# erincatto/solver2d

Measured on AMD Instinct MI355X. Metric: contact-constraints x iters/sec, LargePyramid base-200 TGS_Soft, higher is better.
Workload: dtype f32

## Files before the change

include/solver2d_amd.h:

```cpp
#ifndef SOLVER2D_AMD_H
#define SOLVER2D_AMD_H

#include <stdint.h>

#ifdef __cplusplus
extern "C" {
#endif

#define S2AMD_API_VERSION 5

#define S2AMD_OK 0
#define S2AMD_E_INVALID (-1)
#define S2AMD_E_DEVICE (-2)
#define S2AMD_E_NODEVICE (-3)
#define S2AMD_E_STATE (-4)
#define S2AMD_E_CAPACITY (-5)

typedef enum s2amdSolverType
{
	s2amd_solverJacobi = 0,
	s2amd_solverPGS = 1,
	s2amd_solverPGS_NGS = 2,
	s2amd_solverPGS_NGS_Block = 3,
	s2amd_solverPGS_Soft = 4,
// ... 235 lines not shown
int s2amd_world_get_tree(s2amdSolver* solver, int32_t bodyType, s2amdTreeNode* nodes, int32_t nodeCapacity, int32_t* root);
int s2amd_world_set_contacts(s2amdSolver* solver, const int32_t* slots, int32_t count, const s2amdContact* contacts, const s2amdPairState* pairs);
int s2amd_world_download(s2amdSolver* solver, s2amdBody* bodies, int32_t bodyCapacity, s2amdContact* contacts, int32_t contactCapacity,
						 s2amdJoint* joints, int32_t jointCapacity, s2amdShape* shapes, int32_t shapeCapacity, s2amdPairState* pairs, float* origins,
						 int32_t* status);

int s2amd_find_islands(s2amdSolver* solver, const s2amdBody* bodies, int32_t bodyCapacity, const s2amdContact* contacts, int32_t contactCapacity,
					   const s2amdJoint* joints, int32_t jointCapacity, int32_t* islandOfBody, int32_t* islandCount);
int s2amd_color_constraints(s2amdSolver* solver, const s2amdBody* bodies, int32_t bodyCapacity, const s2amdContact* contacts, int32_t contactCapacity,
							int32_t* colorOfContact, int32_t* colorCount, int32_t* rounds);

int s2amd_export_poses(s2amdSolver* solver, void* devicePoses, int32_t capacity);
int s2amd_export_poses_async(s2amdSolver* solver, void* devicePoses, int32_t capacity, int32_t slot);
int s2amd_export_bodies_async(s2amdSolver* solver, void* deviceRecords, int32_t capacity, int32_t slot);
int s2amd_export_wait(s2amdSolver* solver, int32_t slot);

int s2amd_device_alloc(s2amdSolver* solver, uint64_t bytes, void** devicePtr);
int s2amd_device_free(s2amdSolver* solver, void* devicePtr);
int s2amd_device_read(s2amdSolver* solver, void* hostDst, const void* deviceSrc, uint64_t bytes);

int s2amd_get_contact_order(s2amdSolver* solver, int32_t* order, int32_t orderCapacity, int32_t* colorOffsets,
							int32_t colorCapacity, int32_t* constraintCount, int32_t* colorCount);
int s2amd_get_joint_order(s2amdSolver* solver, int32_t* order, int32_t orderCapacity, int32_t* colorOffsets,
						  int32_t colorCapacity, int32_t* jointCount, int32_t* colorCount);
int s2amd_get_writable_bodies(s2amdSolver* solver, uint8_t* writable, int32_t bodyCapacity, int32_t* solverClass);
int s2amd_get_stats(s2amdSolver* solver, s2amdStepStats* stats);
int s2amd_get_strip_owners(s2amdSolver* solver, int32_t* ownerStrip, int32_t* onSeam, int32_t capacity, int32_t* stripCount);
#define S2AMD_RESIDENT_NONE 0
#define S2AMD_RESIDENT_INTERPRETER 1
#define S2AMD_RESIDENT_ISLAND 2
#define S2AMD_RESIDENT_WIDE 3
#define S2AMD_RESIDENT_WIDE_ONLY_LAUNCH 4
int s2amd_get_resident_kernel(s2amdSolver* solver, int32_t* kernel, int32_t* rounds);
int s2amd_variant_family_count(void);
int s2amd_get_variant_family(int32_t family, const char** kernel, const char** keyFields, int32_t* keyLength, int32_t* entryCount);
int s2amd_get_variant_entry(int32_t family, int32_t entry, int32_t* key, int32_t keyCapacity, uint64_t* selections);
int s2amd_measure_dominant(s2amdSolver* solver, const s2amdStepParams* params, int32_t repeats, float* usPerLaunch,
						   int32_t* launchesPerSweep, int32_t* constraintsPerLaunch);
int s2amd_set_option(s2amdSolver* solver, const char* key, int32_t value);

typedef struct s2amdShardedSolver s2amdShardedSolver;
int s2amd_sharded_create(const int32_t* devices, int32_t deviceCount, s2amdShardedSolver** out);
void s2amd_sharded_destroy(s2amdShardedSolver* sharded);
int s2amd_sharded_shard_count(const s2amdShardedSolver* sharded);
s2amdSolver* s2amd_sharded_solver(s2amdShardedSolver* sharded, int32_t shard);
int s2amd_sharded_upload(s2amdShardedSolver* sharded, const s2amdBody* bodies, int32_t bodyCapacity, const s2amdContact* contacts, int32_t contactCapacity,
						 const s2amdJoint* joints, int32_t jointCapacity);
int s2amd_sharded_step(s2amdShardedSolver* sharded, const s2amdStepParams* params);
int s2amd_sharded_step_async(s2amdShardedSolver* sharded, const s2amdStepParams* params);
int s2amd_sharded_wait(s2amdShardedSolver* sharded);
int s2amd_sharded_get_step_ops(s2amdShardedSolver* sharded, int32_t* streamOps, int32_t* hostWaits, int32_t* exchange);
int s2amd_sharded_count_ops(int32_t shards, int32_t exchange, int32_t* streamOps);
int s2amd_sharded_download(s2amdShardedSolver* sharded, s2amdBody* bodies, int32_t bodyCapacity, s2amdContact* contacts, int32_t contactCapacity,
						   s2amdJoint* joints, int32_t jointCapacity);
int s2amd_sharded_read_bodies(s2amdShardedSolver* sharded, int32_t shard, float* records, int32_t bodyCapacity);
int s2amd_sharded_reshard(s2amdShardedSolver* sharded, const s2amdContact* contacts, int32_t contactCapacity, const s2amdJoint* joints, int32_t jointCapacity);
int s2amd_sharded_get_partition(s2amdShardedSolver* sharded, int32_t* shardOfBody, int32_t capacity, int32_t* islandCount, int32_t* reshards);

#ifdef __cplusplus
}
#endif

#endif
```

solver2d_amd/csrc/solver.cpp:

```cpp

#include <atomic>
#include "solver_executor.h"

namespace
{

thread_local std::string g_lastError;
thread_local std::string g_variantMiss;

}

void s2amdVariantMiss(const char* family, const char* fields, const int* key, int n)
{
	if (!g_variantMiss.empty())
	{
		return;
	}
	std::string text = std::string("no ") + family + " variant for {" + fields + "} = {";
	for (int i = 0; i < n; ++i)
	{
		text += (i != 0 ? ", " : "") + std::to_string(key[i]);
	}
	g_variantMiss = text + "}: nothing was launched for that part of the world";
}
// ... 656 lines not shown
	}
	if (entryCount)
	{
		*entryCount = f[family].entries;
	}
	return S2AMD_OK;
}

int s2amd_get_variant_entry(int32_t family, int32_t entry, int32_t* key, int32_t keyCapacity, uint64_t* selections)
{
	VariantFamily f[S2_VARIANT_FAMILIES];
	if (family < 0 || family >= variantFamilies(f) || entry < 0 || entry >= f[family].entries)
	{
		return fail(S2AMD_E_INVALID, "variant family or entry out of range");
	}
	if (key != nullptr && keyCapacity < f[family].keyLength)
	{
		return fail(S2AMD_E_CAPACITY, "key buffer too small");
	}
	int k[S2_VARIANT_KEY_MAX];
	unsigned long long n = 0;
	f[family].read(f[family].list, entry, k, &n);
	for (int i = 0; key != nullptr && i < f[family].keyLength; ++i)
	{
		key[i] = k[i];
	}
	if (selections)
	{
		*selections = n;
	}
	return S2AMD_OK;
}

int s2amd_get_strip_owners(s2amdSolver* s, int32_t* ownerStrip, int32_t* onSeam, int32_t capacity, int32_t* stripCount)
{
	if (!s)
	{
		return fail(S2AMD_E_INVALID, "null solver");
	}
	const IncrementalStrips& m = s->stripInc;
	const int nb = s->bodyCapacity;
	if ((ownerStrip || onSeam) && capacity < nb)
	{
		return fail(S2AMD_E_CAPACITY, "strip owner buffer too small");
	}
	if (stripCount)
	{
		*stripCount = m.valid ? (int)m.stripBodyCount.size() : 0;
	}
	for (int i = 0; i < nb; ++i)
	{
		if (ownerStrip)
		{
			ownerStrip[i] = (m.valid && i < (int)m.ownerStrip.size()) ? m.ownerStrip[(size_t)i] : -1;
		}
		if (onSeam)
		{
			onSeam[i] = -1;
		}
	}
	if (onSeam && m.valid)
	{
		for (size_t sm = 0; sm < m.seamGroupOf.size(); ++sm)
		{
			const int g = m.seamGroupOf[sm];
			if (g < 0)
// ... 353 lines not shown
		s->structureDirty = true;
	}
	else if (strcmp(key, "persist_debug") == 0)
	{
		s->stripsRejected = false;
		s->optPersistDebug = value;
		s->structureDirty = true;
	}
	else if (strcmp(key, "seam_regs") == 0)
	{
		s->optSeamRegs = value != 0;
		s->structureDirty = true;
	}
	else if (strcmp(key, "wide") == 0)
	{
		s->optWide = value != 0;
		s->structureDirty = true;
	}
	else if (strcmp(key, "pair_lanes") == 0)
	{
		s->optPairLanes = value != 0;
		s->structureDirty = true;
	}
	else if (strcmp(key, "strip_slack") == 0)
	{
		s->optStripSlack = value != 0;
		s->structureDirty = true;
	}
	else if (strcmp(key, "strip_retry") == 0)
	{
		s->optStripRetry = value != 0;
		s->structureDirty = true;
	}
	else if (strcmp(key, "persist") == 0)
	{
		s->stripsRejected = false;
		s->optPersist = value != 0;
		s->structureDirty = true;
	}
	else if (strcmp(key, "strip_patience") == 0)
	{
		s->optStripPatience = std::max(0, value);
		s->stripPatienceNow = s->optStripPatience;
		s->stripPatienceSet = true;
	}
	else if (strcmp(key, "near_handoff") == 0)
	{
		s->optNearHandoff = value != 0;
		s->nearHandoffNow = s->optNearHandoff;
	}
	else if (strcmp(key, "strip_adopt") == 0)
	{
		s->optStripAdopt = value != 0;
	}
	else if (strcmp(key, "prebuild_solver") == 0)
	{
		s->optPrebuildSolver = value;
	}
	else if (strcmp(key, "jacobi_persist") == 0)
	{
		s->optJacobiPersist = value != 0;
		s->structureDirty = true;
	}
	else if (strcmp(key, "jacobi_min_constraints") == 0)
	{
		s->optJacobiMinConstraints = std::max(0, value);
// ... 127 lines not shown
```

solver2d_amd/csrc/solver_async.cpp:

```cpp
#include "solver_internal.h"

#include <atomic>
#include <mutex>
#include <thread>

namespace
{
struct DevPool
{
	std::mutex m;
	std::vector<std::pair<void*, size_t>> blocks;
	size_t bytes = 0;
	std::vector<hipStream_t> streams;
	std::vector<std::pair<void*, size_t>> pinned;
};
constexpr int kMaxPoolDevices = 64;
DevPool& devPool()
{
	static DevPool pools[kMaxPoolDevices];
	int device = 0;
	if (hipGetDevice(&device) != hipSuccess || device < 0 || device >= kMaxPoolDevices)
	{
		(void)hipGetLastError();
		device = 0;
// ... 632 lines not shown
	{
		return false;
	}
	if (job->dropped)
	{
		return false;
	}
	const long due = job->requestedAtStep + (long)job->delay;
	if (s->stepCounter < due)
	{
		return false;
	}
	if (job->forced && !job->done.load(std::memory_order_acquire))
	{
		job->delay += 4;
		return false;
	}
	const double t0 = nowMs();
	const double ta0 = t0;
	if (job->worker.joinable())
	{
		job->worker.join();
	}
	s->asyncWaitMs += (float)(nowMs() - t0);
	s2amdSolver* c = job->clone;
	bool ok = job->rc == S2AMD_OK && job->solverType == solverType && !c->structureDirty;
	auto score = [](const s2amdSolver* x) {
		if (x->dStripA.view.groupCount == 0)
		{
			return 0;
		}
		if (x->persistValid && x->persist.maxRoundsA <= S2_STRIP_ROUNDS)
		{
			return (x->persist.maxRoundsA <= 5 && x->persist.maxSeamRounds <= 2) ? 4 : 3;
		}
		return x->persistValid ? 2 : 1;
	};
	if (ok && job->search)
	{
		if (score(c) <= score(s))
		{
			ok = false;
			if (c->stripScaleFound > 0.0f && c->stripScaleFoundFor == s->stripScaleFoundFor)
			{
				s->stripScaleFound = c->stripScaleFound;
			}
		}
		else
		{
			s->stripSearchPause = 256, s->stripSearchNotBefore = 0;
		}
	}
	const bool poolWas = devPoolOn();
	devPoolThread(true);
	ok = ok && replay(c, job->log);
	if (ok && c->watchedCount > 0)
	{
		if (fetchPointCounts(s) != S2AMD_OK)
		{
			ok = false;
		}
		std::vector<ContactChange> flipped;
		for (int i = 0; ok && i < s->contactCapacity; ++i)
		{
			if (c->hContactWatched[(size_t)i] && s->hContactPoints[(size_t)i] > 0 && c->inc.positionOfSlot[(size_t)i] == -1)
			{
				if (c->hContactEdge[(size_t)i] && !c->hContactDead[(size_t)i] && c->stripInc.valid &&
// ... 51 lines not shown
```

solver2d_amd/csrc/solver_internal.h:

```cpp
#pragma once

#include "launch.h"
#include "s2_device.h"

#include "solver2d_amd.h"

#include <algorithm>
#include <chrono>
#include <cmath>
#include <cstdio>
#include <cstdlib>
#include <cstring>
#include <string>
#include <unordered_map>
#include <vector>

int s2amdFail(int code, const std::string& msg);
inline int fail(int code, const std::string& msg) { return s2amdFail(code, msg); }

#define S2_HUB_DEGREE 12
#define S2_COST_STRIP_ROUND_US 1.4f
#define S2_COST_LAUNCH_US 2.0f
#define S2_COST_BATCH_COLOURS 12
#define S2_COST_TAIL_VISIT_US 0.38f
// ... 371 lines not shown
	std::vector<uint8_t> hBodyLive, hBodyStatic;
	DevBuf dOps;
	long placedTotal = 0;
	DevBuf dSeparated;
	DevBuf dPairLog;
	unsigned long long* hostPairLog = nullptr;
	bool pairLogDirty = false;
	DevBuf dShapeBoxes;
	DevBuf dRefitOrder, dStepBack;
	int refitOrderCount = 0;
	int optTreeStream = 1;
	DeviceTrees* trees = nullptr;
	int lastMovedCount = 0;
	DevBuf dSlotBytes;
	std::vector<uint8_t> hSlotBytes;
	bool slotBytesFresh = false;
	std::vector<int32_t> hSeparated;
	int optIncremental = 1;
	int optDefer = 1;
	int optIslandResident = 1;
	int optStripLean = 1;
	int optStageJoints = 1;
	int optSelfContained = 1;
	int optGeneric = 1;
	int optFreeBodyGroups = 1;
	int optPersist = 1;
	int optSeamRegs = 1;
	int optWide = 1;
	int optWideBodyWarm = 0;
	int optSelfContainedStrips = 0;
	int optStripSlack = 1;
	int optPairLanes = 0;
	int optStripRetry = 1;
	int optPersistDebug = 0;
	int optPersistSpinLimit = 1 << 21;
	bool persistFailed = false;
	int persistFallbacks = 0;
	int optPersistRetry = 256;
	int persistRetryAfter = 256, persistFailedAge = 0;
	int cuCount = 0;
	HubCosts hubCosts;
	unsigned int* hostError = nullptr;
	unsigned long long* hostTimes = nullptr;
	int optMessage = 0;
	int optBodyWarm = 1;
	bool indexInWire = false;
	int graphAge = 0;
	int optStripPatience = 1;
	int optNearHandoff = 1, nearHandoffNow = 1, nearHandoffTimeouts = 0;
	int optStripAdopt = 1;
	int optJacobiPersist = 1;
	int optJacobiMinConstraints = 1024;
	int optOverflow = 1;
	long slicedSteps = 0;
	bool slicedThisStep = false;
	int stripPatienceNow = 1;
	int groupPatienceNow = 0;
	bool dirtyByGroups = false;
	int tailSlackShift = 0;
	bool dirtyByWatched = false;
	int optGroupPatience = 1;
	int optTailTinyColour = 32;
	int optGroupTinyColour = 3;
	int optGenericPlace = 1;
	int optFlipColours = 1;
	bool stripPatienceSet = false;
// ... 166 lines not shown
```

solver2d_amd/csrc/solver_structure.cpp:

```cpp
#include "solver_internal.h"

#include <atomic>

namespace
{

constexpr int ColorBitsWords = 4;

struct Carver
{
	char* p;
	char* end;
	template <class T> T* take(size_t count)
	{
		char* r = p;
		p += (count * sizeof(T) + 255) & ~size_t(255);
		return (T*)r;
	}
};

int growFamily(s2amdSolver* s, DevBuf& buf, int& cap, int need, size_t slotBytes, int arrays)
{
	if (need <= cap && buf.p != nullptr)
	{
// ... 382 lines not shown
	return S2AMD_OK;
}

struct LocalSlots
{
	std::vector<int> slot, stamp;
	int epoch = 0;
	explicit LocalSlots(int nb) : slot((size_t)nb, -1), stamp((size_t)nb, -1) {}
	void begin() { epoch += 1; }
	void seed(int body, std::vector<int>& ids, bool owned)
	{
		stamp[body] = epoch;
		slot[body] = (int)ids.size();
		ids.push_back((int)((uint32_t)body | (owned ? S2G_OWNED : 0u)));
	}
	int get(int body, std::vector<int>& ids, const std::vector<uint8_t>& conflict)
	{
		if (stamp[body] != epoch)
		{
			stamp[body] = epoch;
			slot[body] = (int)ids.size();
			ids.push_back((int)((uint32_t)body | (conflict[body] ? S2G_OWNED : 0u)));
		}
		return slot[body];
	}
};

struct StripPartition
{
	bool active = false;
	std::vector<std::vector<int>> bodies;
	std::vector<std::vector<int>> cA, jA;
	std::vector<std::vector<int>> cB, jB;
};

void partitionStrips(const EdgeList& ce, const EdgeList& je, const std::vector<int>& cGlobal, const std::vector<int>& jGlobal,
					 const std::vector<uint8_t>& conflict, const std::vector<uint8_t>& loose, int nb, int targetBodies, int maxBodies,
					 StripPartition& out)
{
	auto linked = [&](int a, int b) { return a >= 0 && b >= 0 && conflict[a] && conflict[b] && loose[a] && loose[b]; };
	std::vector<int> deg((size_t)nb + 1, 0);
	auto countEdges = [&](const EdgeList& e, const std::vector<int>& ks) {
		for (int k : ks)
		{
			if (linked(e.a[k], e.b[k]))
			{
				deg[(size_t)e.a[k] + 1] += 1;
				deg[(size_t)e.b[k] + 1] += 1;
			}
		}
	};
	countEdges(ce, cGlobal);
	countEdges(je, jGlobal);
	for (int i = 0; i < nb; ++i)
	{
		deg[(size_t)i + 1] += deg[i];
	}
	std::vector<int> adj((size_t)deg[nb]), cursor(deg.begin(), deg.end() - 1);
	auto fillEdges = [&](const EdgeList& e, const std::vector<int>& ks) {
		for (int k : ks)
		{
			if (linked(e.a[k], e.b[k]))
			{
				adj[(size_t)cursor[e.a[k]]++] = e.b[k];
				adj[(size_t)cursor[e.b[k]]++] = e.a[k];
			}
		}
	};
	fillEdges(ce, cGlobal);
	fillEdges(je, jGlobal);

	std::vector<int> level((size_t)nb, -1), queue, levelOffsets{0}, levelBodies;
	std::vector<int> seen((size_t)nb, 0);
	int epoch = 0;
	auto bfs = [&](int root, bool record) {
		epoch += 1;
		queue.clear();
		queue.push_back(root);
		seen[root] = epoch;
		size_t head = 0, levelEnd = 1;
		while (head < queue.size())
		{
			if (head == levelEnd)
			{
				if (record)
				{
					levelOffsets.push_back((int)levelBodies.size());
				}
				levelEnd = queue.size();
			}
			int u = queue[head++];
			if (record)
			{
				level[u] = (int)levelOffsets.size() - 1;
				levelBodies.push_back(u);
			}
			for (int e = deg[u]; e < deg[(size_t)u + 1]; ++e)
			{
				int v = adj[(size_t)e];
				if (seen[v] != epoch)
				{
					seen[v] = epoch;
					queue.push_back(v);
				}
			}
		}
		if (record)
		{
			levelOffsets.push_back((int)levelBodies.size());
		}
		return queue.back();
	};
	for (int i = 0; i < nb; ++i)
	{
		if (!loose[i] || level[i] >= 0)
		{
			continue;
		}
		int far = deg[(size_t)i + 1] > deg[i] ? bfs(i, false) : i;
		bfs(far, true);
	}
	const int levels = (int)levelOffsets.size() - 1;
	if (levels < 4)
	{
		return;
	}

	std::vector<int> stripOf((size_t)nb, -1);
	int curLevels = 0;
	out.bodies.emplace_back();
	for (int l = 0; l < levels; ++l)
	{
		if (curLevels >= 2 && (int)out.bodies.back().size() >= targetBodies)
		{
			out.bodies.emplace_back();
			curLevels = 0;
		}
		for (int e = levelOffsets[l]; e < levelOffsets[(size_t)l + 1]; ++e)
		{
			out.bodies.back().push_back(levelBodies[(size_t)e]);
		}
		curLevels += 1;
	}
	if (curLevels < 2 && out.bodies.size() >= 2)
	{
		std::vector<int> lastStrip = std::move(out.bodies.back());
		out.bodies.pop_back();
		out.bodies.back().insert(out.bodies.back().end(), lastStrip.begin(), lastStrip.end());
	}
	const int K = (int)out.bodies.size();
	if (K < 2)
	{
		out = StripPartition();
		return;
	}
	for (int i = 0; i < K; ++i)
	{
		for (int body : out.bodies[(size_t)i])
		{
			stripOf[body] = i;
		}
	}

	out.cA.assign((size_t)K, {}), out.jA.assign((size_t)K, {});
	out.cB.assign((size_t)K - 1, {}), out.jB.assign((size_t)K - 1, {});
	bool ok = true;
// ... 887 lines not shown
	s2amdSolver* s;
	const int solverType;
	const float stripScale;
	const int cls;
	const bool needAdj;
	const bool grouped;
	const bool ldsGroups;
	const bool wantStrips;
	const bool residentWanted;
	const bool stripSlackWanted;
	const int nb;
	SweepSet& cs;
	SweepSet& js;

	std::vector<uint8_t> conflict;
	EdgeList ce, je;
	int C = 0, J = 0;
	std::vector<int> cPart, jPart;
	int groupCount = 0;
	std::vector<uint32_t> flags;
	std::vector<std::vector<int>> cOf, jOf;
	StripPartition strips;
	bool stripsNeedOneLaunch = false;
	LocalSlots slots;
	std::vector<int> seamGroup;
	struct SpareRound
	{
		int table, group, begin, count, round;
	};
	std::vector<SpareRound> spareRounds;
	int stripBaseC = 0;
	int overflowBase = 0, overflowCount = 0;
	bool rebuild = false;

	double t0, tPhase;
	bool prepTimes;
	double tSlots = 0, tColour = 0, tAppend = 0;

	StructureBuild(s2amdSolver* solver, int type, float scale)
		: s(solver), solverType(type), stripScale(scale), cls(isPositionSolver(type) ? 1 : 0), needAdj(type == s2amd_solverJacobi),
		  grouped(solver->optGroups != 0 && !needAdj),
		  ldsGroups(grouped && (solver->optGroupPatience == 0 || solver->graphAge >= solver->groupPatienceNow)),
		  wantStrips(grouped && solver->optStrips != 0 && !solver->stripsRejected && solver->graphAge >= solver->stripPatienceNow &&
					 (solver->optStripsAnySolver != 0 || isSoftFamily(type) || genericWanted(solver))),
		  residentWanted(grouped && isSoftFamily(type) && solver->optIslandResident != 0 && !solver->residentRejected),
		  stripSlackWanted(solver->optStripSlack != 0 && solver->optIncremental != 0 && solver->optPersist != 0 &&
						   (type == s2amd_solverTGS_Soft || (solver->optWide != 0 && (type == s2amd_solverSoftStep || type == s2amd_solverPGS_Soft)) ||
							(!isSoftFamily(type) && solver->optGenericPlace != 0 && genericWanted(solver)))),
		  nb(solver->bodyCapacity),
		  cs(solver->contacts), js(solver->joints), slots(solver->bodyCapacity)
	{
		static const bool fromEnv = getenv("S2AMD_DEBUG_PREP") != nullptr;
		prepTimes = fromEnv;
		t0 = tPhase = nowMs();
	}

	static bool genericWanted(const s2amdSolver* solver)
	{
		return solver->optGeneric != 0 && solver->optPersist != 0 && solver->optStripLean != 0 && !solver->persistFailed && solver->hostError != nullptr;
	}

	static int stripBodiesFor(const s2amdSolver* solver, int type)
	{
		const bool ldsSeams = (type == s2amd_solverSoftStep || type == s2amd_solverPGS_Soft) && solver->optWide == 0;
		if (solver->stripBodiesSet || !ldsSeams)
		{
// ... 265 lines not shown
			for (int k = 0; k < J; ++k)
			{
				jPart[k] = assign(jRoot[k]);
			}
		}

		phase("islands and groups");
	}

	void splitParts()
	{
		cOf.assign((size_t)groupCount + 1, {}), jOf.assign((size_t)groupCount + 1, {});
		for (int k = 0; k < C; ++k)
		{
			cOf[(size_t)cPart[k] + 1].push_back(k);
		}
		for (int k = 0; k < J; ++k)
		{
			jOf[(size_t)jPart[k] + 1].push_back(k);
		}

		cs = SweepSet();
		js = SweepSet();
		cs.colorOffsets.push_back(0);
		js.colorOffsets.push_back(0);
		s->hGroups.clear();
		s->hResident.clear();
		s->hContactTail.clear();
		s->hJointTail.clear();
		s->hStripA.clear();
		s->hStripB.clear();
	}

	void cutStrips()
	{
		strips = StripPartition();
		stripsNeedOneLaunch = false;
		if (wantStrips && (s->optStripsAnySolver != 0 || jOf[0].empty() || genericWanted(s)))
		{
			std::vector<uint8_t> ownedByIsland((size_t)nb, 0);
			auto mark = [&](int body) {
				if (body >= 0 && conflict[body])
				{
					ownedByIsland[body] = 1;
				}
			};
			for (int k = 0; k < C; ++k)
			{
				if (cPart[k] >= 0)
				{
					mark(ce.a[k]), mark(ce.b[k]);
				}
			}
			for (int k = 0; k < J; ++k)
			{
				if (jPart[k] >= 0)
				{
					mark(je.a[k]), mark(je.b[k]);
				}
			}
			std::vector<uint8_t> loose((size_t)nb);
			int looseCount = 0;
			for (int i = 0; i < nb; ++i)
			{
				loose[i] = s->hBodyLive[i] && !s->hBodyStatic[i] && !ownedByIsland[i];
				looseCount += loose[i];
			}
			if (looseCount >= (s->stripMinBodiesSet || s->maxGroupBodiesSet ? s->optStripMinBodies : std::min(s->optStripMinBodies, groupLowerLimit(solverType))))
			{
				partitionStrips(ce, je, cOf[0], jOf[0], conflict, loose, nb, std::max(8, (int)((float)stripBodiesFor(s, solverType) * stripScale)), s->optMaxGroupBodies, strips);
			}
			if (strips.active)
			{
				std::vector<uint8_t> placed((size_t)nb, 0);
				for (const std::vector<int>& list : strips.bodies)
				{
					for (int b : list)
					{
						placed[(size_t)b] = 1;
					}
				}
				bool unfit = false;
				for (const std::vector<std::vector<int>>* lists : {&strips.cA, &strips.cB})
				{
					for (const std::vector<int>& list : *lists)
					{
						for (int k : list)
						{
							unfit = unfit || (ce.a[k] >= 0 && conflict[(size_t)ce.a[k]] && !placed[(size_t)ce.a[k]]) ||
									 (ce.b[k] >= 0 && conflict[(size_t)ce.b[k]] && !placed[(size_t)ce.b[k]]);
						}
					}
				}
				for (const std::vector<std::vector<int>>* lists : {&strips.jA, &strips.jB})
				{
					for (const std::vector<int>& list : *lists)
					{
						for (int k : list)
						{
							unfit = unfit || (je.a[k] >= 0 && conflict[(size_t)je.a[k]] && !placed[(size_t)je.a[k]]) ||
									 (je.b[k] >= 0 && conflict[(size_t)je.b[k]] && !placed[(size_t)je.b[k]]);
						}
					}
// ... 563 lines not shown
		}
		if ((rc = uploadGroupTable(s, s->hGroups, s->dGroups)) != 0 || (rc = uploadGroupTable(s, s->hContactTail, s->dContactTail, s->hContactTail.count() > 0 ? (size_t)(S2_TAIL_BODY_SLACK << s->tailSlackShift) : 0)) != 0 ||
			(rc = uploadGroupTable(s, s->hJointTail, s->dJointTail)) != 0 ||
			(rc = uploadGroupTable(s, s->hStripA, s->dStripA, s->hStripA.count() > 0 ? (size_t)32 * (size_t)(s->hStripA.maxBodies + S2_STRIP_ADOPT_SLACK) : 0)) != 0 ||
			(rc = uploadGroupTable(s, s->hStripB, s->dStripB)) != 0)
		{
			return rc;
		}
		phase("index tables");
		return S2AMD_OK;
	}

	int buildStripTables()
	{
		int rc;
		s->leanAValid = s->leanBValid = false;
		s->persistValid = false;
		s->leanA = StripTableView{};
		s->leanB = StripTableView{};
		if (strips.active && s->optStripLean)
		{
			if ((rc = buildLeanStripTables(s, strips, conflict, seamGroup, stripBaseC, nb)) != 0)
			{
				return rc;
			}
		}

		s->stripsNeedOneLaunch = strips.active && stripsNeedOneLaunch;
		if (stripsNeedOneLaunch)
		{
			s->leanAValid = s->leanBValid = false;
		}
		const bool soft = isSoftFamily(solverType);
		const bool oneLaunch = (soft && s->persistValid) || s->genericValid;
		const bool multiLaunch = !stripsNeedOneLaunch && (s->optStripsAnySolver != 0 || (soft && js.stripCount == 0 && s->leanAValid && s->leanBValid));
		if (strips.active && !oneLaunch && !multiLaunch)
		{
			s->stripsRejected = true;
			s->structureDirty = true;
			rebuild = true;
			return S2AMD_OK;
		}
		phase("strip tables");
		buildStripMirror();
		phase("strip mirror");
		return S2AMD_OK;
	}

	void buildStripMirror()
	{
		IncrementalStrips& m = s->stripInc;
		m = IncrementalStrips{};
		const bool interpreter = !isSoftFamily(solverType);
		if (!strips.active || !stripSlackWanted || !(interpreter ? s->genericValid : s->persistValid) || js.stripCount != 0)
		{
			return;
		}
		m.base = stripBaseC, m.end = stripBaseC + cs.stripCount;
		if (interpreter)
		{
			m.takeOnly = true;
			m.roundLimit[0] = m.roundLimit[1] = 0;
		}
		if (solverType == s2amd_solverSoftStep)
		{
			m.roundLimit[0] = S2_STRIP_ROUNDS, m.roundLimit[1] = 2;
// ... 156 lines not shown
		for (size_t k = 0; k < cs.order.size(); ++k)
		{
			s->slackPositions += cs.order[k] < 0 ? 1 : 0;
		}
		s->slackAtBuild = s->slackPositions;
		s->inc.valid = s->optIncremental != 0 && s->inc.solverClass == cls && !s->msgTablesValid && !s->inc.positionOfSlot.empty();
		s->inc.patches.clear();
		s->orderSolverClass = cls;
		s->orderResident = residentWanted;
		s->orderColourless = needAdj;
		s->orderGrouped = grouped;
		s->orderLdsGroups = ldsGroups;
		if (getenv("S2AMD_DEBUG"))
		{
			int real = 0;
			for (int k = 0; k < cs.globalCount; ++k)
			{
				real += cs.order[(size_t)k] >= 0 ? 1 : 0;
			}
			fprintf(stderr, "[s2amd] structure: global part %d contact positions (%d constraints, %d batches%s), %d joints; %d LDS groups, %d resident, %d strips; loose bodies %d\n",
					cs.globalCount, real, (int)cs.batchOffsets.size() - 1, cs.hasTail ? ", tail" : "", js.globalCount, s->hGroups.count(), s->hResident.count(),
					s->hStripA.count(), s->looseBodies);
		}
		s->residentAllTwoPoints = residentAllTwoPoints(s) ? 1 : 0;
		s->orderStrips = wantStrips;
		s->orderStripBodies = stripBodiesFor(s, solverType);
		s->structureDirty = false;
		s->structureGeneration += 1;
		s->stats.hostPrepMs = (float)(nowMs() - t0);
		return S2AMD_OK;
	}
};

static int buildStructureWith(s2amdSolver* s, int solverType, float stripScale)
{
	StructureBuild build(s, solverType, stripScale);
	if (build.upToDate())
	{
		return S2AMD_OK;
	}
	if (s->worldResident && !s->pointsKnown)
	{
		int rcDead = syncDeadSlots(s);
		if (rcDead)
		{
			return rcDead;
		}
	}
	int rc = build.gatherEdges();
	if (rc)
	{
		return rc;
	}
	build.findIslands();
	build.splitParts();
	build.cutStrips();
	build.phase("strip partition");
	build.colourGlobalPart();
	build.phase("global part");
	build.emitIslandGroups();
	build.emitStrips();
	if ((rc = build.uploadTables()) != 0 || build.rebuild || (rc = build.buildStripTables()) != 0 || build.rebuild)
	{
		return rc ? rc : buildStructureWith(s, solverType, stripScale);
	}
	return build.finish();
}

int buildStructure(s2amdSolver* s, int solverType)
{
	if (asyncBuildsOn(s) && s->optAsyncBuild >= 2 && !s->structureDirty)
	{
		StructureBuild probe(s, solverType, 1.0f);
		if (probe.onlyStripsMissing())
		{
			return asyncRequest(s, solverType, false);
		}
	}
	const uint64_t before = s->structureGeneration;
	{
		const int cls = isPositionSolver(solverType) ? 1 : 0;
		if (s->stripsJudgedForClass != cls)
		{
			s->stripsRejected = s->stripsHopeless = false;
			s->stripsJudgedForClass = cls;
		}
	}
	if (s->stripScaleFoundFor != StructureBuild::stripBodiesFor(s, solverType))
	{
		s->stripScaleFound = 0.0f;
		s->stripScaleFoundFor = StructureBuild::stripBodiesFor(s, solverType);
	}
	const float firstScale = s->stripScaleFound > 0.0f ? s->stripScaleFound : 1.0f;
	int rc = buildStructureWith(s, solverType, firstScale);
	if (rc != S2AMD_OK || s->structureGeneration == before || s->optStripRetry == 0)
	{
		return rc;
	}
	auto outcome = [&]() {
		if (s->persistValid && !s->persist.wideRounds)
		{
			return (s->persist.maxRoundsA <= 5 && s->persist.maxSeamRounds <= 2) ? 3 : 2;
		}
		return (s->persistValid || (s->leanAValid && s->leanBValid)) ? 1 : 0;
	};
	auto satisfied = [&]() {
		if (!StructureBuild::isSoftFamily(solverType))
		{
			return s->dStripA.view.groupCount > 0 && (s->genericValid || outcome() >= 1);
		}
		if (s->joints.stripCount > 0)
		{
			return s->dStripA.view.groupCount > 0 && s->genericValid;
		}
		return outcome() >= (solverType == s2amd_solverTGS_Soft ? 3 : 2);
	};
	const bool triedStrips = s->stripsRejected || s->dStripA.view.groupCount > 0;
	s->stripRetryPending = false;
	auto usable = [&]() { return s->dStripA.view.groupCount > 0 && s->persistValid && s->stripInc.valid; };
	if (s->forcedBuild && (usable() || !triedStrips || s->stripsHopeless))
	{
		return rc;
	}
	if (!s->forcedBuild && (!triedStrips || s->stripsHopeless || satisfied() || (s->stripScaleFound > 0.0f && outcome() >= 2)))
	{
		return rc;
	}
	if (!s->forcedBuild && s->optStripPatience != 0 && s->graphAge < 32)
	{
		s->stripRetryPending = true;
		return rc;
	}
	float bestScale = firstScale;
	int best = outcome();
	const float scales[] = {4.0f, 10.0f, 20.0f, 2.0f, 40.0f, 80.0f, 0.5f};
// ... 29 lines not shown
```

solver2d_amd/hip.py:

```python
import ctypes
import os

import numpy as np

from . import wire

_HERE = os.path.dirname(os.path.abspath(__file__))
LIB_PATH = os.environ.get("S2AMD_LIB") or os.path.join(_HERE, "libs2amd.so")
FAST_LIB_PATH = os.environ.get("S2AMD_FAST_LIB") or os.path.join(_HERE, "libs2amd_fast.so")

EXPORTS = [
    "s2amd_api_version", "s2amd_build_flags", "s2amd_device_count", "s2amd_device_bus_id", "s2amd_last_error", "s2amd_create", "s2amd_destroy",
    "s2amd_solve", "s2amd_upload", "s2amd_step_resident", "s2amd_download", "s2amd_save_bodies",
    "s2amd_restore_bodies", "s2amd_get_contact_order", "s2amd_get_joint_order", "s2amd_get_writable_bodies", "s2amd_get_stats",
    "s2amd_set_option", "s2amd_export_poses", "s2amd_export_poses_async", "s2amd_export_bodies_async", "s2amd_export_wait", "s2amd_measure_dominant", "s2amd_refit_shapes", "s2amd_find_pairs", "s2amd_synchronize", "s2amd_update_contacts", "s2amd_find_islands", "s2amd_color_constraints",
    "s2amd_world_upload", "s2amd_world_step", "s2amd_world_download", "s2amd_world_find_pairs", "s2amd_world_set_contacts",
    "s2amd_device_alloc", "s2amd_device_free", "s2amd_device_read", "s2amd_world_separated", "s2amd_world_download_boxes", "s2amd_world_set_refit_order", "s2amd_world_download_step", "s2amd_world_set_tree", "s2amd_world_get_tree",
    "s2amd_get_strip_owners", "s2amd_get_resident_kernel", "s2amd_variant_family_count", "s2amd_get_variant_family", "s2amd_get_variant_entry",
    "s2amd_sharded_create", "s2amd_sharded_destroy", "s2amd_sharded_shard_count", "s2amd_sharded_solver", "s2amd_sharded_upload", "s2amd_sharded_step",
    "s2amd_sharded_download", "s2amd_sharded_read_bodies", "s2amd_sharded_reshard", "s2amd_sharded_get_partition",
    "s2amd_sharded_step_async", "s2amd_sharded_wait", "s2amd_sharded_get_step_ops", "s2amd_sharded_count_ops",
]

_libs = {}


class S2AmdError(RuntimeError):
    pass


def load(fast=False):
    path = FAST_LIB_PATH if fast else LIB_PATH
    if path in _libs:
        return _libs[path]
    if not os.path.exists(path):
        raise S2AmdError("HIP extension %s is missing: build it with `make -C solver2d_amd/csrc` "
                         "(there is no CPU fallback)" % path)
    L = ctypes.CDLL(path)
    vp, i32 = ctypes.c_void_p, ctypes.c_int32
    L.s2amd_api_version.restype = ctypes.c_int
    L.s2amd_device_count.restype = ctypes.c_int
    L.s2amd_last_error.restype = ctypes.c_char_p
    L.s2amd_build_flags.restype = ctypes.c_char_p
    L.s2amd_create.argtypes = [ctypes.c_int, ctypes.POINTER(vp)]
    L.s2amd_destroy.argtypes = [vp]
    L.s2amd_destroy.restype = None
    L.s2amd_solve.argtypes = [vp, ctypes.POINTER(wire.StepParams), vp, i32, vp, i32, vp, i32]
    L.s2amd_upload.argtypes = [vp, vp, i32, vp, i32, vp, i32]
    L.s2amd_step_resident.argtypes = [vp, ctypes.POINTER(wire.StepParams)]
    L.s2amd_download.argtypes = [vp, vp, i32, vp, i32, vp, i32]
    L.s2amd_save_bodies.argtypes = [vp]
    L.s2amd_restore_bodies.argtypes = [vp]
    L.s2amd_synchronize.argtypes = [vp]
    L.s2amd_get_contact_order.argtypes = [vp, vp, i32, vp, i32, ctypes.POINTER(i32), ctypes.POINTER(i32)]
    L.s2amd_get_joint_order.argtypes = [vp, vp, i32, vp, i32, ctypes.POINTER(i32), ctypes.POINTER(i32)]
    L.s2amd_get_writable_bodies.argtypes = [vp, vp, i32, ctypes.POINTER(i32)]
    L.s2amd_get_strip_owners.argtypes = [vp, vp, vp, i32, ctypes.POINTER(i32)]
    L.s2amd_get_resident_kernel.argtypes = [vp, ctypes.POINTER(i32), ctypes.POINTER(i32)]
    L.s2amd_variant_family_count.restype = ctypes.c_int
    L.s2amd_get_variant_family.argtypes = [i32, ctypes.POINTER(ctypes.c_char_p), ctypes.POINTER(ctypes.c_char_p), ctypes.POINTER(i32), ctypes.POINTER(i32)]
    L.s2amd_get_variant_entry.argtypes = [i32, i32, ctypes.POINTER(i32), i32, ctypes.POINTER(ctypes.c_uint64)]
    L.s2amd_get_stats.argtypes = [vp, ctypes.POINTER(wire.StepStats)]
    L.s2amd_set_option.argtypes = [vp, ctypes.c_char_p, i32]
    L.s2amd_export_poses.argtypes = [vp, vp, i32]
    L.s2amd_export_poses_async.argtypes = [vp, vp, i32, i32]
    L.s2amd_export_bodies_async.argtypes = [vp, vp, i32, i32]
    L.s2amd_export_wait.argtypes = [vp, i32]
    L.s2amd_measure_dominant.argtypes = [vp, ctypes.POINTER(wire.StepParams), i32, ctypes.POINTER(ctypes.c_float),
                                         ctypes.POINTER(i32), ctypes.POINTER(i32)]
    L.s2amd_refit_shapes.argtypes = [vp, vp, i32, vp, i32, vp]
    L.s2amd_find_pairs.argtypes = [vp, vp, i32, vp, i32, vp, vp, i32, vp, i32, vp, i32, ctypes.POINTER(i32)]
    L.s2amd_update_contacts.argtypes = [vp, vp, i32, vp, vp, i32, vp, vp, i32, vp]
    L.s2amd_world_upload.argtypes = [vp, vp, i32, vp, i32, vp, i32, vp, i32, vp, vp]
    L.s2amd_world_step.argtypes = [vp, ctypes.POINTER(wire.StepParams), ctypes.POINTER(wire.WorldStepInfo)]
    L.s2amd_world_find_pairs.argtypes = [vp, vp, i32, ctypes.POINTER(i32)]
    L.s2amd_world_set_contacts.argtypes = [vp, vp, i32, vp, vp]
    L.s2amd_world_separated.argtypes = [vp, vp, i32, ctypes.POINTER(i32)]
    L.s2amd_world_download_boxes.argtypes = [vp, vp, i32]
    L.s2amd_world_set_refit_order.argtypes = [vp, vp, i32]
    L.s2amd_world_set_tree.argtypes = [vp, i32, vp, i32, i32]
    L.s2amd_world_get_tree.argtypes = [vp, i32, vp, i32, ctypes.POINTER(i32)]
    L.s2amd_world_download.argtypes = [vp, vp, i32, vp, i32, vp, i32, vp, i32, vp, vp, vp]
    L.s2amd_device_alloc.argtypes = [vp, ctypes.c_uint64, ctypes.POINTER(vp)]
    L.s2amd_device_free.argtypes = [vp, vp]
    L.s2amd_device_read.argtypes = [vp, vp, vp, ctypes.c_uint64]
    L.s2amd_find_islands.argtypes = [vp, vp, i32, vp, i32, vp, i32, vp, ctypes.POINTER(i32)]
    L.s2amd_color_constraints.argtypes = [vp, vp, i32, vp, i32, vp, ctypes.POINTER(i32), ctypes.POINTER(i32)]
    L.s2amd_sharded_create.argtypes = [vp, i32, ctypes.POINTER(vp)]
    L.s2amd_sharded_destroy.argtypes = [vp]
    L.s2amd_sharded_destroy.restype = None
    L.s2amd_sharded_shard_count.argtypes = [vp]
# ... 283 lines not shown
        existing = np.ascontiguousarray(existing, dtype=np.int32).reshape(-1, 2)
        moved = np.ascontiguousarray(moved, dtype=np.uint8)
        cap = 4096
        while True:
            out = np.zeros((cap, 2), dtype=np.int32)
            n = ctypes.c_int32()
            rc = self._L.s2amd_find_pairs(self._h, wire.as_ptr(bodies), len(bodies), wire.as_ptr(shapes), len(shapes), wire.as_ptr(moved),
                                         wire.as_ptr(existing), len(existing), wire.as_ptr(joints), len(joints), wire.as_ptr(out), cap,
                                         ctypes.byref(n))
            if rc == -5 and n.value > cap:
                cap = n.value
                continue
            self._ck(rc)
            return out[: n.value].copy()

    def _order(self, fn):
        n, nc = ctypes.c_int32(), ctypes.c_int32()
        self._ck(fn(self._h, None, 0, None, 0, ctypes.byref(n), ctypes.byref(nc)))
        order = np.zeros(max(n.value, 1), dtype=np.int32)
        offsets = np.zeros(nc.value + 1, dtype=np.int32)
        self._ck(fn(self._h, order.ctypes.data, len(order), offsets.ctypes.data, len(offsets), ctypes.byref(n), ctypes.byref(nc)))
        return order[: n.value].copy(), offsets

    def contact_order(self):
        return self._order(self._L.s2amd_get_contact_order)

    def strip_owners(self, body_capacity):
        owner = np.full(max(body_capacity, 1), -1, dtype=np.int32)
        seam = np.full(max(body_capacity, 1), -1, dtype=np.int32)
        n = ctypes.c_int32()
        self._ck(self._L.s2amd_get_strip_owners(self._h, owner.ctypes.data, seam.ctypes.data, len(owner), ctypes.byref(n)))
        return owner[:body_capacity], seam[:body_capacity], n.value

    def resident_kernel(self):
        kernel, rounds = ctypes.c_int32(), ctypes.c_int32()
        self._ck(self._L.s2amd_get_resident_kernel(self._h, ctypes.byref(kernel), ctypes.byref(rounds)))
        return kernel.value, rounds.value

    def joint_order(self):
        return self._order(self._L.s2amd_get_joint_order)

    def synchronize(self):
        self._ck(self._L.s2amd_synchronize(self._h))

    def stats(self):
        st = wire.StepStats()
        self._ck(self._L.s2amd_get_stats(self._h, ctypes.byref(st)))
        return {k: getattr(st, k) for k, _ in wire.StepStats._fields_}


class _BorrowedSolver(Solver):

    def __init__(self, L, handle):
        self._L, self._h, self.fast = L, ctypes.c_void_p(handle), False

    def close(self):
        self._h = None


class ShardedSolver:

    def __init__(self, devices, fast=False):
        L = load(fast=fast)
        devs = (ctypes.c_int32 * len(devices))(*[int(d) for d in devices])
        h = ctypes.c_void_p()
        _check(L.s2amd_sharded_create(devs, len(devices), ctypes.byref(h)), L)
# ... 70 lines not shown
```

Baseline: 6.294 billion.

## Add opt-in strip cut candidates that minimise interior coloring rounds

Adds an optional search over alternative strip partitions: second BFS root, thin end strips, and level-first constraint ordering. It keeps whichever candidate needs the fewest interior color rounds without adding seam rounds, aiming to cut the per-iteration round count in the persistent soft kernel. The partition scoring also now favours structures with four or fewer interior rounds. The search costs extra host time at structure build and may force a rebuild. A query API for strip rounds is added.

Result: slower. 6.226 billion (-1.1%).

```diff
diff --git a/include/solver2d_amd.h b/include/solver2d_amd.h
--- a/include/solver2d_amd.h
+++ b/include/solver2d_amd.h
@@ -291,6 +291,7 @@
 #define S2AMD_RESIDENT_WIDE 3
 #define S2AMD_RESIDENT_WIDE_ONLY_LAUNCH 4
 int s2amd_get_resident_kernel(s2amdSolver* solver, int32_t* kernel, int32_t* rounds);
+int s2amd_get_strip_rounds(s2amdSolver* solver, int32_t* interior, int32_t* seam);
 int s2amd_variant_family_count(void);
 int s2amd_get_variant_family(int32_t family, const char** kernel, const char** keyFields, int32_t* keyLength, int32_t* entryCount);
 int s2amd_get_variant_entry(int32_t family, int32_t entry, int32_t* key, int32_t keyCapacity, uint64_t* selections);
diff --git a/solver2d_amd/csrc/solver.cpp b/solver2d_amd/csrc/solver.cpp
--- a/solver2d_amd/csrc/solver.cpp
+++ b/solver2d_amd/csrc/solver.cpp
@@ -712,6 +712,33 @@
 	return S2AMD_OK;
 }
 
+int s2amd_get_strip_rounds(s2amdSolver* s, int32_t* interior, int32_t* seam)
+{
+	if (!s)
+	{
+		return fail(S2AMD_E_INVALID, "null solver");
+	}
+	const HostGroupTable* tables[2] = {&s->hStripA, &s->hStripB};
+	int32_t* out[2] = {interior, seam};
+	for (int t = 0; t < 2; ++t)
+	{
+		int most = 0;
+		for (int g = 0; s->dStripA.view.groupCount > 0 && g < tables[t]->count(); ++g)
+		{
+			most = std::max(most, tables[t]->cBatchOffsets[(size_t)g + 1] - tables[t]->cBatchOffsets[(size_t)g]);
+		}
+		if (s->persistValid && s->dStripA.view.groupCount > 0)
+		{
+			most = std::max(most, t == 0 ? s->persist.maxRoundsA : s->persist.maxSeamRounds);
+		}
+		if (out[t])
+		{
+			*out[t] = most;
+		}
+	}
+	return S2AMD_OK;
+}
+
 int s2amd_get_strip_owners(s2amdSolver* s, int32_t* ownerStrip, int32_t* onSeam, int32_t capacity, int32_t* stripCount)
 {
 	if (!s)
@@ -1131,6 +1158,13 @@
 		s->optStripRetry = value != 0;
 		s->structureDirty = true;
 	}
+	else if (strcmp(key, "strip_cuts") == 0)
+	{
+		s->optStripCuts = value != 0;
+		s->structureDirty = true;
+		s->stripsRejected = false;
+		s->stripScaleFound = 0.0f;
+	}
 	else if (strcmp(key, "persist") == 0)
 	{
 		s->stripsRejected = false;
diff --git a/solver2d_amd/csrc/solver_async.cpp b/solver2d_amd/csrc/solver_async.cpp
--- a/solver2d_amd/csrc/solver_async.cpp
+++ b/solver2d_amd/csrc/solver_async.cpp
@@ -688,7 +688,7 @@
 		}
 		if (x->persistValid && x->persist.maxRoundsA <= S2_STRIP_ROUNDS)
 		{
-			return (x->persist.maxRoundsA <= 5 && x->persist.maxSeamRounds <= 2) ? 4 : 3;
+			return x->persist.maxSeamRounds > 2 || x->persist.maxRoundsA > 5 ? 3 : (x->persist.maxRoundsA > 4 ? 4 : 5);
 		}
 		return x->persistValid ? 2 : 1;
 	};
diff --git a/solver2d_amd/csrc/solver_internal.h b/solver2d_amd/csrc/solver_internal.h
--- a/solver2d_amd/csrc/solver_internal.h
+++ b/solver2d_amd/csrc/solver_internal.h
@@ -427,6 +427,7 @@
 	int optStripSlack = 1;
 	int optPairLanes = 0;
 	int optStripRetry = 1;
+	int optStripCuts = 0;
 	int optPersistDebug = 0;
 	int optPersistSpinLimit = 1 << 21;
 	bool persistFailed = false;
diff --git a/solver2d_amd/csrc/solver_structure.cpp b/solver2d_amd/csrc/solver_structure.cpp
--- a/solver2d_amd/csrc/solver_structure.cpp
+++ b/solver2d_amd/csrc/solver_structure.cpp
@@ -438,11 +438,19 @@
 	std::vector<std::vector<int>> bodies;
 	std::vector<std::vector<int>> cA, jA;
 	std::vector<std::vector<int>> cB, jB;
+	std::vector<int> level;
+};
+
+struct StripCut
+{
+	bool secondRoot = false;
+	bool thinEnds = false;
+	int maxStrips = 0;
 };
 
 void partitionStrips(const EdgeList& ce, const EdgeList& je, const std::vector<int>& cGlobal, const std::vector<int>& jGlobal,
 					 const std::vector<uint8_t>& conflict, const std::vector<uint8_t>& loose, int nb, int targetBodies, int maxBodies,
-					 StripPartition& out)
+					 StripPartition& out, const StripCut& cut = StripCut())
 {
 	auto linked = [&](int a, int b) { return a >= 0 && b >= 0 && conflict[a] && conflict[b] && loose[a] && loose[b]; };
 	std::vector<int> deg((size_t)nb + 1, 0);
@@ -477,7 +485,7 @@
 	fillEdges(je, jGlobal);
 
 	std::vector<int> level((size_t)nb, -1), queue, levelOffsets{0}, levelBodies;
-	std::vector<int> seen((size_t)nb, 0);
+	std::vector<int> seen((size_t)nb, 0), dist;
 	int epoch = 0;
 	auto bfs = [&](int root, bool record) {
 		epoch += 1;
@@ -524,8 +532,40 @@
 			continue;
 		}
 		int far = deg[(size_t)i + 1] > deg[i] ? bfs(i, false) : i;
+		if (cut.secondRoot && deg[(size_t)far + 1] > deg[far])
+		{
+			bfs(far, false);
+			dist.resize((size_t)nb, -1);
+			dist[(size_t)far] = 0;
+			for (int u : queue)
+			{
+				for (int e = deg[u]; e < deg[(size_t)u + 1]; ++e)
+				{
+					if (dist[(size_t)adj[(size_t)e]] < 0)
+					{
+						dist[(size_t)adj[(size_t)e]] = dist[(size_t)u] + 1;
+					}
+				}
+			}
+			const int last = dist[(size_t)queue.back()];
+			int root = queue.back();
+			for (size_t q = queue.size(); q-- > 0 && dist[(size_t)queue[q]] == last;)
+			{
+				const int u = queue[q];
+				if (deg[(size_t)u + 1] - deg[u] <= deg[(size_t)root + 1] - deg[root])
+				{
+					root = u;
+				}
+			}
+			for (int u : queue)
+			{
+				dist[(size_t)u] = -1;
+			}
+			far = root;
+		}
 		bfs(far, true);
 	}
+	out.level = level;
 	const int levels = (int)levelOffsets.size() - 1;
 	if (levels < 4)
 	{
@@ -537,7 +577,8 @@
 	out.bodies.emplace_back();
 	for (int l = 0; l < levels; ++l)
 	{
-		if (curLevels >= 2 && (int)out.bodies.back().size() >= targetBodies)
+		const bool thin = cut.thinEnds && (int)out.bodies.size() + (levels - l) / 2 <= cut.maxStrips;
+		if (curLevels >= 2 && ((int)out.bodies.back().size() >= targetBodies || thin))
 		{
 			out.bodies.emplace_back();
 			curLevels = 0;
@@ -1491,6 +1532,8 @@
 	int stripBaseC = 0;
 	int overflowBase = 0, overflowCount = 0;
 	bool rebuild = false;
+	bool tryCuts = true;
+	bool altCut = false;
 
 	double t0, tPhase;
 	bool prepTimes;
@@ -1822,6 +1865,138 @@
 		s->hStripB.clear();
 	}
 
+	bool cutCandidatesWanted() const
+	{
+		return s->optStripCuts != 0 && s->optStripRetry != 0 && !s->stripBodiesSet && isSoftFamily(solverType) && jOf[0].empty() && s->optPersist != 0 && s->optStripLean != 0 &&
+			   s->hostError != nullptr;
+	}
+
+	void stripRounds(const StripPartition& p, int& interior, int& seam, std::vector<int>& local) const
+	{
+		std::vector<int> a, b, color, used;
+		std::vector<uint8_t> lconf;
+		auto rounds = [&](const std::vector<int>& ks) {
+			a.clear(), b.clear(), lconf.clear(), used.clear();
+			auto slot = [&](int body) {
+				if (body < 0)
+				{
+					return -1;
+				}
+				if (local[(size_t)body] < 0)
+				{
+					local[(size_t)body] = (int)lconf.size();
+					lconf.push_back(conflict[(size_t)body]);
+					used.push_back(body);
+				}
+				return local[(size_t)body];
+			};
+			for (int k : ks)
+			{
+				a.push_back(slot(ce.a[k])), b.push_back(slot(ce.b[k]));
+			}
+			const int cc = colorGraph(a, b, lconf, (int)lconf.size(), color, 256);
+			for (int body : used)
+			{
+				local[(size_t)body] = -1;
+			}
+			return cc;
+		};
+		interior = seam = 0;
+		for (const std::vector<int>& ks : p.cA)
+		{
+			interior = std::max(interior, rounds(ks));
+		}
+		for (const std::vector<int>& ks : p.cB)
+		{
+			seam = std::max(seam, rounds(ks));
+		}
+	}
+
+	void orderLevelFirst(StripPartition& p) const
+	{
+		auto cls = [&](int k) {
+			const int a = ce.a[k], b = ce.b[k];
+			if (a < 0 || b < 0 || !conflict[(size_t)a] || !conflict[(size_t)b])
+			{
+				return 2;
+			}
+			return p.level[(size_t)a] != p.level[(size_t)b] ? 0 : 1;
+		};
+		for (std::vector<int>& ks : p.cA)
+		{
+			std::stable_sort(ks.begin(), ks.end(), [&](int x, int y) { return cls(x) < cls(y); });
+		}
+	}
+
+	void chooseCut(const std::vector<uint8_t>& loose, int targetBodies)
+	{
+		const double tc0 = nowMs();
+		const bool debug = getenv("S2AMD_DEBUG") != nullptr;
+		std::vector<int> local((size_t)nb, -1);
+		int baseA = 0, baseB = 0;
+		stripRounds(strips, baseA, baseB, local);
+		if (debug)
+		{
+			fprintf(stderr, "[s2amd] strip cut: default partition, %d strips, %d interior / %d seam rounds\n", (int)strips.bodies.size(), baseA, baseB);
+		}
+		if (baseB > 2)
+		{
+			if (debug)
+			{
+				fprintf(stderr, "[s2amd] strip cut: default partition kept (more than two seam rounds: no candidates)\n");
+			}
+			return;
+		}
+		StripPartition best;
+		int bestA = baseA, bestB = baseB;
+		for (int c = 1; c < 8 && baseA > 1; ++c)
+		{
+			const bool levelFirst = (c & 1) != 0;
+			StripCut cut;
+			cut.thinEnds = (c & 2) != 0, cut.secondRoot = (c & 4) != 0;
+			cut.maxStrips = s->cuCount;
+			StripPartition p;
+			if (c == 1)
+			{
+				p = strips;
+			}
+			else
+			{
+				partitionStrips(ce, je, cOf[0], jOf[0], conflict, loose, nb, targetBodies, s->optMaxGroupBodies, p, cut);
+			}
+			if (!p.active || (int)p.bodies.size() > s->cuCount)
+			{
+				continue;
+			}
+			if (levelFirst)
+			{
+				orderLevelFirst(p);
+			}
+			int rA = 0, rB = 0;
+			stripRounds(p, rA, rB, local);
+			if (debug)
+			{
+				fprintf(stderr, "[s2amd] strip cut: candidate%s%s%s, %d strips, %d interior / %d seam rounds\n", cut.secondRoot ? " second-root" : "",
+						cut.thinEnds ? " thin-ends" : "", levelFirst ? " level-first" : "", (int)p.bodies.size(), rA, rB);
+			}
+			if (rA < bestA && rB <= baseB)
+			{
+				bestA = rA, bestB = rB;
+				best = std::move(p);
+			}
+		}
+		if (best.active)
+		{
+			strips = std::move(best);
+			altCut = true;
+		}
+		if (debug)
+		{
+			fprintf(stderr, "[s2amd] strip cut: %s (%d interior / %d seam rounds), %.3f ms of host time\n", altCut ? "candidate adopted" : "default partition kept", bestA,
+					bestB, nowMs() - tc0);
+		}
+	}
+
 	void cutStrips()
 	{
 		strips = StripPartition();
@@ -1858,7 +2033,12 @@
 			}
 			if (looseCount >= (s->stripMinBodiesSet || s->maxGroupBodiesSet ? s->optStripMinBodies : std::min(s->optStripMinBodies, groupLowerLimit(solverType))))
 			{
-				partitionStrips(ce, je, cOf[0], jOf[0], conflict, loose, nb, std::max(8, (int)((float)stripBodiesFor(s, solverType) * stripScale)), s->optMaxGroupBodies, strips);
+				const int targetBodies = std::max(8, (int)((float)stripBodiesFor(s, solverType) * stripScale));
+				partitionStrips(ce, je, cOf[0], jOf[0], conflict, loose, nb, targetBodies, s->optMaxGroupBodies, strips);
+				if (strips.active && tryCuts && cutCandidatesWanted())
+				{
+					chooseCut(loose, targetBodies);
+				}
 			}
 			if (strips.active)
 			{
@@ -2488,6 +2668,12 @@
 			s->leanAValid = s->leanBValid = false;
 		}
 		const bool soft = isSoftFamily(solverType);
+		if (altCut && !s->persistValid)
+		{
+			s->structureDirty = true;
+			rebuild = true;
+			return S2AMD_OK;
+		}
 		const bool oneLaunch = (soft && s->persistValid) || s->genericValid;
 		const bool multiLaunch = !stripsNeedOneLaunch && (s->optStripsAnySolver != 0 || (soft && js.stripCount == 0 && s->leanAValid && s->leanBValid));
 		if (strips.active && !oneLaunch && !multiLaunch)
@@ -2710,9 +2896,10 @@
 	}
 };
 
-static int buildStructureWith(s2amdSolver* s, int solverType, float stripScale)
+static int buildStructureWith(s2amdSolver* s, int solverType, float stripScale, bool tryCuts = true)
 {
 	StructureBuild build(s, solverType, stripScale);
+	build.tryCuts = tryCuts;
 	if (build.upToDate())
 	{
 		return S2AMD_OK;
@@ -2740,7 +2927,7 @@
 	build.emitStrips();
 	if ((rc = build.uploadTables()) != 0 || build.rebuild || (rc = build.buildStripTables()) != 0 || build.rebuild)
 	{
-		return rc ? rc : buildStructureWith(s, solverType, stripScale);
+		return rc ? rc : buildStructureWith(s, solverType, stripScale, tryCuts && !build.altCut);
 	}
 	return build.finish();
 }
@@ -2778,7 +2965,7 @@
 	auto outcome = [&]() {
 		if (s->persistValid && !s->persist.wideRounds)
 		{
-			return (s->persist.maxRoundsA <= 5 && s->persist.maxSeamRounds <= 2) ? 3 : 2;
+			return s->persist.maxSeamRounds > 2 || s->persist.maxRoundsA > 5 ? 2 : (s->persist.maxRoundsA > 4 ? 3 : 4);
 		}
 		return (s->persistValid || (s->leanAValid && s->leanBValid)) ? 1 : 0;
 	};
diff --git a/solver2d_amd/hip.py b/solver2d_amd/hip.py
--- a/solver2d_amd/hip.py
+++ b/solver2d_amd/hip.py
@@ -16,7 +16,7 @@
     "s2amd_set_option", "s2amd_export_poses", "s2amd_export_poses_async", "s2amd_export_bodies_async", "s2amd_export_wait", "s2amd_measure_dominant", "s2amd_refit_shapes", "s2amd_find_pairs", "s2amd_synchronize", "s2amd_update_contacts", "s2amd_find_islands", "s2amd_color_constraints",
     "s2amd_world_upload", "s2amd_world_step", "s2amd_world_download", "s2amd_world_find_pairs", "s2amd_world_set_contacts",
     "s2amd_device_alloc", "s2amd_device_free", "s2amd_device_read", "s2amd_world_separated", "s2amd_world_download_boxes", "s2amd_world_set_refit_order", "s2amd_world_download_step", "s2amd_world_set_tree", "s2amd_world_get_tree",
-    "s2amd_get_strip_owners", "s2amd_get_resident_kernel", "s2amd_variant_family_count", "s2amd_get_variant_family", "s2amd_get_variant_entry",
+    "s2amd_get_strip_owners", "s2amd_get_strip_rounds", "s2amd_get_resident_kernel", "s2amd_variant_family_count", "s2amd_get_variant_family", "s2amd_get_variant_entry",
     "s2amd_sharded_create", "s2amd_sharded_destroy", "s2amd_sharded_shard_count", "s2amd_sharded_solver", "s2amd_sharded_upload", "s2amd_sharded_step",
     "s2amd_sharded_download", "s2amd_sharded_read_bodies", "s2amd_sharded_reshard", "s2amd_sharded_get_partition",
     "s2amd_sharded_step_async", "s2amd_sharded_wait", "s2amd_sharded_get_step_ops", "s2amd_sharded_count_ops",
@@ -57,6 +57,7 @@
     L.s2amd_get_writable_bodies.argtypes = [vp, vp, i32, ctypes.POINTER(i32)]
     L.s2amd_get_strip_owners.argtypes = [vp, vp, vp, i32, ctypes.POINTER(i32)]
     L.s2amd_get_resident_kernel.argtypes = [vp, ctypes.POINTER(i32), ctypes.POINTER(i32)]
+    L.s2amd_get_strip_rounds.argtypes = [vp, ctypes.POINTER(i32), ctypes.POINTER(i32)]
     L.s2amd_variant_family_count.restype = ctypes.c_int
     L.s2amd_get_variant_family.argtypes = [i32, ctypes.POINTER(ctypes.c_char_p), ctypes.POINTER(ctypes.c_char_p), ctypes.POINTER(i32), ctypes.POINTER(i32)]
     L.s2amd_get_variant_entry.argtypes = [i32, i32, ctypes.POINTER(i32), i32, ctypes.POINTER(ctypes.c_uint64)]
@@ -406,6 +407,11 @@
         self._ck(self._L.s2amd_get_strip_owners(self._h, owner.ctypes.data, seam.ctypes.data, len(owner), ctypes.byref(n)))
         return owner[:body_capacity], seam[:body_capacity], n.value
 
+    def strip_rounds(self):
+        interior, seam = ctypes.c_int32(), ctypes.c_int32()
+        self._ck(self._L.s2amd_get_strip_rounds(self._h, ctypes.byref(interior), ctypes.byref(seam)))
+        return interior.value, seam.value
+
     def resident_kernel(self):
         kernel, rounds = ctypes.c_int32(), ctypes.c_int32()
         self._ck(self._L.s2amd_get_resident_kernel(self._h, ctypes.byref(kernel), ctypes.byref(rounds)))
```
